# felixlutz/carla-social-force-model

Hardware: AMD Instinct MI355X
Metric: sfm_ticks_per_s (higher is better)
Workload: dtype f32

## Files before the change

### carla-social-force-model_amd/_lib.py

```python
from __future__ import annotations

import ctypes as C
import os

import numpy as np

PKG_DIR = os.path.dirname(os.path.abspath(__file__))
LIB_PATH = os.environ.get("SFM_LIB_PATH") or os.path.join(PKG_DIR, "libsfm_hip.so")
ABI_VERSION = 17
SINCE = {"sfm_step_packed": 4, "sfm_set_dynamic_obstacles_packed": 4, "sfm_step_records": 5,
         **{n: 6 for n in ("sfm_batch_create", "sfm_batch_destroy", "sfm_batch_set_stream", "sfm_batch_set_params",
                           "sfm_batch_upload_state", "sfm_batch_set_borders", "sfm_batch_set_static_obstacles",
                           "sfm_batch_set_dynamic_obstacles", "sfm_batch_tick", "sfm_batch_run", "sfm_batch_download_state",
                           "sfm_batch_last_error")},
         **{n: 7 for n in ("sfm_batch_set_waypoint_streams", "sfm_batch_download_waypoints", "sfm_batch_run_recorded")},
         **{n: 8 for n in ("sfm_batch_set_dynamic_boxes", "sfm_batch_download_dynamic_obstacles")},
         **{n: 9 for n in ("sfm_batch_set_mode_fsm", "sfm_batch_download_modes")},
         **{n: 10 for n in ("sfm_batch_tick_forces", "sfm_batch_run_recorded_forces")},
         **{n: 11 for n in ("sfm_batch_set_spawn_schedule", "sfm_batch_download_spawns")},
         **{n: 12 for n in ("sfm_batch_set_vehicle_tracks", "sfm_batch_download_vehicle_tracks")},
         **{n: 13 for n in ("sfm_batch_snapshot", "sfm_batch_restart")},
         **{n: 14 for n in ("sfm_batch_set_steering", "sfm_batch_set_commands", "sfm_batch_download_steering",
                            "sfm_batch_device_ptr")},
         **{n: 15 for n in ("sfm_batch_set_observation", "sfm_batch_observe", "sfm_batch_download_observations",
# ... 40 lines not shown
    "sfm_destroy": (C.c_int, [_H]),
    "sfm_set_params": (C.c_int, [_H, C.POINTER(SfmParamsC)]),
    "sfm_set_stream": (C.c_int, [_H, C.c_void_p]),
    "sfm_set_borders": (C.c_int, [_H, C.c_int, _I, _F, _F, _F, _F, _F]),
    "sfm_set_static_obstacles": (C.c_int, [_H, C.c_int, _I, _F, _F, _F, _F]),
    "sfm_set_dynamic_obstacles": (C.c_int, [_H, C.c_int, _I, _F, _F, _F, _F, _F, _F]),
    "sfm_set_dynamic_boxes": (C.c_int, [_H, C.c_int, _I, _F, _F, _F, _F, _F, _F, _F, _F]),
    "sfm_download_dynamic_obstacles": (C.c_int, [_H, _F, _F, _F, _F]),
    "sfm_upload_state": (C.c_int, [_H, C.c_int, _F, _F, _F, _F, _F, _F, _F, _F, _F, _F, _U8]),
    "sfm_set_shard": (C.c_int, [_H, C.c_int, C.c_int]),
    "sfm_set_waypoint_stream": (C.c_int, [_H, C.c_uint32, C.c_float, C.c_float]),
    "sfm_set_mode_fsm": (C.c_int, [_H, C.c_int, _U8, _F, _F, _F, _F, _F, _I, _F, _F, _U8, C.c_int, C.c_float, _F]),
    "sfm_download_modes": (C.c_int, [_H, _U8, _F, _I]),
    "sfm_tick": (C.c_int, [_H, C.c_uint32]),
    "sfm_run": (C.c_int, [_H, C.c_int, C.c_uint32]),
    "sfm_run_recorded": (C.c_int, [_H, C.c_int, C.c_uint32, C.c_int, _F, C.c_int, C.POINTER(C.c_int)]),
    "sfm_download_velocities": (C.c_int, [_H, _F, _F, _F]),
    "sfm_step_packed": (C.c_int, [_H, C.c_int, _F, _F, C.c_uint32, _F]),
    "sfm_step_records": (C.c_int, [_H, C.c_int, C.c_void_p, C.c_int64, _I, _U8, C.c_float, C.c_uint32, _F, C.POINTER(C.c_int32)]),
    "sfm_set_dynamic_obstacles_packed": (C.c_int, [_H, C.c_int, _I, _F, _F]),
    "sfm_download_state": (C.c_int, [_H, _F, _F, _F, _F, _F, _F, _F, _F]),
    "sfm_download_forces": (C.c_int, [_H, C.c_int, _F, _F, _F]),
    "sfm_get_arrived": (C.c_int, [_H, C.c_float, _U8]),
    "sfm_download_draw_counts": (C.c_int, [_H, _U32]),
    "sfm_packed_state_ptr": (C.c_void_p, [_H, C.POINTER(C.c_int)]),
    "sfm_packed_z_ptr": (C.c_void_p, [_H]),
    "sfm_row_data_ptr": (C.c_void_p, [_H, C.c_int, C.POINTER(C.c_int)]),
    "sfm_resort": (C.c_int, [_H]),
    "sfm_last_error": (C.c_char_p, [_H]),
    "sfm_get_timing": (C.c_int, [_H, C.POINTER(C.c_float), C.POINTER(C.c_int), C.POINTER(C.c_int)]),
    "sfm_set_timing": (C.c_int, [_H, C.c_int]),
    "sfm_profile_dominant_kernel": (C.c_int, [_H, C.c_int, C.POINTER(C.c_float)]),
    "sfm_kernel_variant": (C.c_char_p, [_H]),
    "sfm_get_pair_work": (C.c_int, [_H, C.POINTER(C.c_longlong), C.POINTER(C.c_longlong)]),
    "sfm_set_partition": (C.c_int, [_H, C.c_int, C.c_int, _I]),
    "sfm_tick_begin": (C.c_int, [_H, C.c_uint32]),
    "sfm_tick_end": (C.c_int, [_H, C.c_uint32]),
    "sfm_batch_create": (C.c_int, [C.c_int, C.POINTER(SfmParamsC), C.c_int, C.POINTER(_H)]),
    "sfm_batch_destroy": (C.c_int, [_H]),
    "sfm_batch_set_stream": (C.c_int, [_H, C.c_void_p]),
    "sfm_batch_set_params": (C.c_int, [_H, C.POINTER(SfmParamsC)]),
    "sfm_batch_upload_state": (C.c_int, [_H, _I, _F, _F, _F, _F, _F, _F, _F, _F, _F, _F, _U8]),
    "sfm_batch_set_borders": (C.c_int, [_H, _I, _I, _F, _F, _F, _F, _F]),
    "sfm_batch_set_static_obstacles": (C.c_int, [_H, _I, _I, _F, _F, _F, _F]),
    "sfm_batch_set_dynamic_obstacles": (C.c_int, [_H, _I, _I, _F, _F, _F, _F, _F, _F]),
    "sfm_batch_tick": (C.c_int, [_H, C.c_uint32]),
    "sfm_batch_run": (C.c_int, [_H, C.c_int, C.c_uint32]),
    "sfm_batch_download_state": (C.c_int, [_H, _F, _F, _F, _F, _F, _F]),
    "sfm_batch_last_error": (C.c_char_p, [_H]),
    "sfm_batch_set_waypoint_streams": (C.c_int, [_H, _U32, _F, _F]),
    "sfm_batch_download_waypoints": (C.c_int, [_H, _F, _F, _U32]),
    "sfm_batch_run_recorded": (C.c_int, [_H, C.c_int, C.c_uint32, C.c_int, _F, _F, C.c_int, C.POINTER(C.c_int)]),
    "sfm_batch_set_dynamic_boxes": (C.c_int, [_H, _I, _I, _F, _F, _F, _F, _F, _F, _F, _F]),
    "sfm_batch_download_dynamic_obstacles": (C.c_int, [_H, _F, _F, _F, _F]),
    "sfm_batch_set_mode_fsm": (C.c_int, [_H, _U8, _F, _F, _F, _F, _F, _I, _F, _F, _U8, _I, _F, _F, _F]),
    "sfm_batch_download_modes": (C.c_int, [_H, _U8, _F, _I, _F]),
    "sfm_batch_tick_forces": (C.c_int, [_H, C.c_uint32, C.c_uint32, _F]),
    "sfm_batch_run_recorded_forces": (C.c_int, [_H, C.c_int, C.c_uint32, C.c_int, C.c_uint32, _F, _F, _F, C.c_int,
                                                C.POINTER(C.c_int)]),
    "sfm_batch_set_spawn_schedule": (C.c_int, [_H, _F, _U8]),
    "sfm_batch_download_spawns": (C.c_int, [_H, _U8, _F]),
    "sfm_batch_set_vehicle_tracks": (C.c_int, [_H, _I, _I, _F, _F, _F, _F, _F, _F]),
    "sfm_batch_download_vehicle_tracks": (C.c_int, [_H, C.POINTER(C.c_int64), _U8]),
    "sfm_batch_snapshot": (C.c_int, [_H]),
    "sfm_batch_restart": (C.c_int, [_H, _U8]),
    "sfm_batch_set_steering": (C.c_int, [_H, _U8, _F, _F, _F]),
# ... 87 lines not shown
```

### carla-social-force-model_amd/csrc/sfm_capi.hip

```cpp
#include "sfm_capi_common.h"

using namespace sfm;

constexpr int GEO_SLICES_MAX = 16;


struct DevGeo {
    DevBuf<int> off;
    DevBuf<float2> pts;
    DevBuf<float4> ctr;
    DevBuf<float4> seg;
    int K = 0;
    int P = 0;
    PinnedBuf<char> stage;
    std::vector<int> off_host;
    bool lazy = false;
    bool lazy_off = false;
};

struct FsmDev {
    bool on = false;
    int n = 0;
    DevBuf<uint8_t> mode;
    DevBuf<float> target, initial, crossing, margin, next;
// ... 98 lines not shown
    FusedDev fused;
    int pair_geo_mode = -1;
    int fused_mode = -1;
    bool hosted = false;
    PinnedBuf<char> down_stage;
    std::vector<float> step_cols;
    std::vector<uint8_t> step_mask;
    bool used_fused = false;
    unsigned long long api_seq = 0, carry_seq = 0;
    bool carry_ok = false;
    int carry_sl = 0;
    bool last_list = false;

    uint32_t seed = 0;
    float world_side = 0.f, arrive_thr = 2.0f;

    FsmDev fsm;

    Event ev0, ev1;
    Stream aux;
    Event ev_fork, ev_join;
    bool overlap_geo = true;
    bool geo_ahead = false;
    DevBuf<uint32_t> work2;
    bool begin_done = false, begin_forked = false, last_split = false;
    int begin_geo_slices = 0;
    uint32_t begin_flags = 0;
    int timed_ticks = 0, timed_launches = 0;
    bool timing_valid = false;
    bool timing_on = true;
    int ipw_last = 0;
    int ipw_override = 0, team_override = 0;
    char variant[64] = "none";
};

static int fail(SfmHandle* h, int code, const char* msg) {
    if (h) h->err = msg; else g_create_error = msg;
    return code;
}

static int bind(SfmHandle* h) {
    if (!h) return SFM_ERR_INVALID;
    ++h->api_seq;
    hipError_t e = hipSetDevice(h->device);
    if (e != hipSuccess) { h->err = std::string("hipSetDevice: ") + hipGetErrorString(e); return SFM_ERR_HIP; }
    return SFM_OK;
}

static void drop_geo_ahead(SfmHandle* h) {
    if (h && h->geo_ahead) {
        hipStreamSynchronize(h->aux);
        h->geo_ahead = false;
    }
    if (h) h->begin_done = false;
}


extern "C" {

int sfm_abi_version(void) { return SFM_ABI_VERSION; }

int sfm_create(const SfmParams* params, int device_id, SfmHandle** out) {
    if (!out) return fail(nullptr, SFM_ERR_INVALID, "out is NULL");
    *out = nullptr;
    const char* why = nullptr;
    if (!check_params(params, &why)) return fail(nullptr, SFM_ERR_INVALID, why);
    int ndev = 0;
    hipError_t e = hipGetDeviceCount(&ndev);
    if (e != hipSuccess || ndev <= 0) return fail(nullptr, SFM_ERR_NO_DEVICE, "no HIP device visible (libsfm_hip needs an MI355X)");
    if (device_id < 0 || device_id >= ndev) return fail(nullptr, SFM_ERR_INVALID, "device_id out of range");
    e = hipSetDevice(device_id);
    if (e != hipSuccess) return fail(nullptr, SFM_ERR_HIP, hipGetErrorString(e));
    SfmHandle* h = new SfmHandle();
    h->device = device_id;
    h->prm = *params;
    if (h->ev0.create() != hipSuccess || h->ev1.create() != hipSuccess) {
        delete h;
        return fail(nullptr, SFM_ERR_HIP, "hipEventCreate failed");
    }
    if (h->aux.create(hipStreamNonBlocking) != hipSuccess || h->ev_fork.create(hipEventDisableTiming) != hipSuccess ||
        h->ev_join.create(hipEventDisableTiming) != hipSuccess) {
        h->aux.reset();
        h->overlap_geo = false;
    }
    const char* ov = getenv("SFM_IPW");
    if (ov) h->ipw_override = atoi(ov);
    ov = getenv("SFM_TEAM");
    if (ov) h->team_override = atoi(ov);
    ov = getenv("SFM_SYM");
    if (ov) h->sym_mode = atoi(ov);
    ov = getenv("SFM_CUTOFF");
    if (ov) h->cut_mode = atoi(ov);
    ov = getenv("SFM_PAIR_GEO");
    if (ov) h->pair_geo_mode = atoi(ov);
    ov = getenv("SFM_FUSED");
    if (ov) h->fused_mode = atoi(ov);
    ov = getenv("SFM_REORDER");
    if (ov) h->reorder_mode = atoi(ov);
    ov = getenv("SFM_GEO_SLICES");
    if (ov) h->geo_slices_override = std::min(GEO_SLICES_MAX, std::max(1, atoi(ov)));
    ov = getenv("SFM_STRIPS");
    if (ov) h->strips_override = atoi(ov) != 0 ? 1 : 0;
    ov = getenv("SFM_RESORT_EVERY");
    if (ov) { h->resort_every = atoi(ov); h->resort_every_set = true; }
    h->dpp_dir = probe_dpp_direction(nullptr);
    *out = h;
    return SFM_OK;
}

int sfm_destroy(SfmHandle* h) {
    if (!h) return SFM_OK;
    hipSetDevice(h->device);
    hipStreamSynchronize(h->stream);
    if (h->aux) hipStreamSynchronize(h->aux);
    delete h;
    return SFM_OK;
}

int sfm_set_params(SfmHandle* h, const SfmParams* params) {
    if (!h) return SFM_ERR_INVALID;
    const char* why = nullptr;
    if (!check_params(params, &why)) return fail(h, SFM_ERR_INVALID, why);
    drop_geo_ahead(h);
    h->carry_ok = false;
    h->prm = *params;
    return SFM_OK;
}

int sfm_set_stream(SfmHandle* h, void* hip_stream) {
// ... 603 lines not shown
    return sa;
}

constexpr int PHASE_FULL = 0, PHASE_BEGIN = 1, PHASE_END = 2;
constexpr int LIST_ALL = 0, LIST_OWN = 1, LIST_REMOTE = 2;

static int fused_launch(SfmHandle* h, uint32_t flags, int mode, int* sl) {
    const int n_g = (h->n_t + 1) / 2;
    const size_t rows = (size_t)n_g * (size_t)h->N_pad;
    TickArgs a;
    fill_args(h, a, flags);
    const bool geo = a.geo != nullptr;
    int slices = 0, nw = 16;
    const int n_pair = fused_pair_workgroups(n_g);
    if (geo) {
        slices = h->n_t <= 64 ? 4 : 2;
        if (h->n_t >= 6) slices = std::max(slices, std::min(FUSED_GEO_SLICES_MAX, (256 - n_pair) / h->n_t));
        if (n_pair + h->n_t * slices > 512) nw = 8;
    }
    const size_t grow = (size_t)FUSED_GEO_SLICES_MAX * (size_t)h->N_pad;
    if (geo && a.adv.M > 0) {
        float4* c_in = mode ? h->fused.dyn_ctr_alt : h->dynamics.ctr;
        float2* p_in = mode ? h->fused.dyn_pts_alt : h->dynamics.pts;
        a.dynamics.ctr = c_in; a.dynamics.pts = p_in;
        a.adv.ctr = c_in; a.adv.pts = p_in;
        a.adv.ctr_out = mode ? h->dynamics.ctr : h->fused.dyn_ctr_alt;
        a.adv.pts_out = mode ? h->dynamics.pts : h->fused.dyn_pts_alt;
    }
    const FusedArgs f{h->fused.fslab + (size_t)(*sl ^ 1) * rows, h->fused.fslab + (size_t)*sl * rows,
                      h->z3 ? h->fused.fslabz + (size_t)(*sl ^ 1) * rows : nullptr, h->z3 ? h->fused.fslabz + (size_t)*sl * rows : nullptr,
                      h->own, h->fused.own_alt, n_g, h->n_t, n_g % 8 == 0 ? 1 : 0,
                      geo ? h->fused.fgeo + (size_t)(*sl ^ 1) * grow : nullptr, geo ? h->fused.fgeo + (size_t)*sl * grow : nullptr, slices,
                      geo ? h->n_t * slices : 0, n_pair, mode};
    HIP_TRY(h, launch_fused_tick(h->rad, a, f, h->stream, nw));
    if (mode != 0) {
        h->cur ^= 1;
        swap(h->own, h->fused.own_alt);
        if (geo && a.adv.M > 0) {
            swap(h->dynamics.ctr, h->fused.dyn_ctr_alt);
            swap(h->dynamics.pts, h->fused.dyn_pts_alt);
        }
    }
    *sl ^= 1;
    return SFM_OK;
}

static int fused_reserve(SfmHandle* h) {
    const size_t need = (size_t)2 * (size_t)((h->n_t + 1) / 2) * (size_t)h->N_pad;
    FusedDev& f = h->fused;
    if (need > f.fslab.cap()) HIP_TRY(h, f.fslab.alloc(need));
    if (h->z3 && need > f.fslabz.cap()) HIP_TRY(h, f.fslabz.alloc(need));
    if (f.own_alt.cap() < (size_t)h->cap) HIP_TRY(h, f.own_alt.alloc((size_t)h->cap));
    const size_t gneed = (size_t)2 * FUSED_GEO_SLICES_MAX * (size_t)h->N_pad;
    if (gneed > f.fgeo.cap()) HIP_TRY(h, f.fgeo.alloc(gneed));
    if (h->dyn_boxes && h->dynamics.K > 0) {
        if (f.dyn_ctr_alt.cap() != h->dynamics.ctr.cap()) HIP_TRY(h, f.dyn_ctr_alt.alloc(h->dynamics.ctr.cap()));
        if (f.dyn_pts_alt.cap() != h->dynamics.pts.cap()) HIP_TRY(h, f.dyn_pts_alt.alloc(h->dynamics.pts.cap()));
    }
    return SFM_OK;
}

static int run_fused(SfmHandle* h, int ticks, uint32_t flags, bool carry, bool geo) {
    int rc = fused_reserve(h);
    if (rc) return rc;
    snprintf(h->variant, sizeof(h->variant), geo ? "sfm_fused_tick_kernel(geo)" : "sfm_fused_tick_kernel");
    if (h->timing_on) HIP_TRY(h, hipEventRecord(h->ev0, h->stream));
    int sl = carry ? h->carry_sl : 0;
// ... 655 lines not shown
    int rc = bind(h);
    if (rc) return rc;
    if (!h->pk[0]) return fail(h, SFM_ERR_STATE, "sfm_upload_state has not been called");
    if (!h->reordered || h->N == 0) return SFM_OK;
    if (h->fsm.on && !(h->i_begin == 0 && h->i_end == h->N))
        return fail(h, SFM_ERR_STATE, "sfm_resort on a shard with the device-side mode state machine");
    return resort_rows(h);
}

const char* sfm_last_error(const SfmHandle* h) { return h ? h->err.c_str() : g_create_error.c_str(); }

int sfm_set_timing(SfmHandle* h, int enable) {
    if (!h) return SFM_ERR_INVALID;
    h->carry_ok = false;
    h->timing_on = enable != 0;
    if (!h->timing_on) h->timing_valid = false;
    return SFM_OK;
}

int sfm_get_timing(SfmHandle* h, float* elapsed_ms, int* ticks, int* launches) {
    int rc = bind(h);
    if (rc) return rc;
    if (!h->timing_valid) return fail(h, SFM_ERR_STATE, h->timing_on ? "no timed run yet" : "timing is switched off (sfm_set_timing)");
    HIP_TRY(h, hipEventSynchronize(h->ev1));
    float ms = 0.f;
    HIP_TRY(h, hipEventElapsedTime(&ms, h->ev0, h->ev1));
    if (elapsed_ms) *elapsed_ms = ms;
    if (ticks) *ticks = h->timed_ticks;
    if (launches) *launches = h->timed_launches;
    return SFM_OK;
}

const char* sfm_kernel_variant(const SfmHandle* h) { return h ? h->variant : "none"; }

int sfm_get_pair_work(SfmHandle* h, long long* tile_pair_items, long long* pair_terms) {
    int rc = bind(h);
    if (rc) return rc;
    if (!h->pk[0]) return fail(h, SFM_ERR_STATE, "sfm_upload_state has not been called");
    if (!h->used_sym) return fail(h, SFM_ERR_STATE, "the last tick did not run the symmetric pair kernel");
    HIP_TRY(h, hipStreamSynchronize(h->stream));
    const long long t_own = (h->i_end + WAVE - 1) / WAVE - h->i_begin / WAVE;
    long long items, diag_items = (t_own + 1) / 2;
    if (h->last_list) {
        int cnt[4] = {0, 0, 0, 0};
        HIP_TRY(h, hipMemcpy(cnt, h->work_count, sizeof(int) * 4, hipMemcpyDeviceToHost));
        items = (h->count_zeroed ? cnt[2] : cnt[0]) + (h->last_split ? (h->count_zeroed ? cnt[3] : cnt[1]) : 0);
    } else {
        const long long n_t = h->n_t;
        items = n_t * (n_t - 1) / 2 + diag_items;
    }
    if (tile_pair_items) *tile_pair_items = items;
    if (pair_terms) *pair_terms = (items - diag_items) * (long long)(WAVE * WAVE) + t_own * (long long)(WAVE * WAVE / 2);
    return SFM_OK;
}

}
```

### carla-social-force-model_amd/csrc/sfm_capi_common.h

```cpp
#pragma once
#include "sfm_devbuf.h"
#include "sfm_device.h"
#include "sfm_hip.h"

#include <algorithm>
#include <cmath>
#include <numeric>
#include <cstdio>
#include <cstdlib>
#include <cstring>
#include <limits>
#include <string>
#include <vector>

namespace sfm {
hipError_t launch_tick(int ipw, int team, bool z3, bool rad, const TickArgs& a, hipStream_t st);
hipError_t launch_arrived(const float4* pk, const float4* own, int N, float thr2, uint8_t* mask, hipStream_t st);
hipError_t launch_sym_list(const TickArgs& a, const SymArgs& sa, hipStream_t st, int partners = 0, bool count_is_zero = false);
hipError_t launch_sym_pair(bool rad, const TickArgs& a, const SymArgs& sa, hipStream_t st);
hipError_t launch_sym_epilogue(bool rad, const TickArgs& a, const SymArgs& sa, hipStream_t st);
hipError_t launch_fused_tick(bool rad, const TickArgs& a, const FusedArgs& f, hipStream_t st, int waves);
int fused_pair_workgroups(int n_g);
hipError_t launch_sym_pair_geo(bool rad, const TickArgs& a, const SymArgs& sa, hipStream_t st);
int sym_item_count(int n_t);
hipError_t launch_strip_bounds(const float4* box, const float* vmax, int n_t, int tps, int n_strips, float4* sbox, float* svmax,
                               hipStream_t st);
hipError_t launch_tile_strip_bounds(const float4* pk, int N, int n_t, int tps, int n_strips, float4* box, float* vmax, float4* sbox,
                                    float* svmax, hipStream_t st);
hipError_t launch_geometry(bool rad, const TickArgs& a, hipStream_t st);
hipError_t launch_modes(const TickArgs& a, hipStream_t st);
struct ReorderBufs { unsigned long long *key64_in, *key64_out; uint32_t *row_a, *row_b, *key32_in, *key32_out; void* temp; size_t temp_bytes; };
size_t reorder_temp_bytes(int N);
hipError_t launch_resort(const float4* pk, int N, int strip_rows, const ReorderBufs& b, hipStream_t st);
hipError_t launch_resort_blocks(const float4* pk, int N, const BlockPlan& pl, const ReorderBufs& b, hipStream_t st);
hipError_t launch_unpack_geo(const char* block, float4* ctr, int K, float2* pts, int P, int* off, bool with_off, hipStream_t st);
hipError_t launch_unpack_rows(const char* block, size_t b_own, size_t b_zv, size_t b_rr, size_t b_cm, int n_pad, float4* pk0,
                              float4* pk1, float4* own, float2* zv0, float2* zv1, float* radius, uint8_t* crossing, uint32_t* draws,
                              const char* geo_block, float4* ctr, int K, float2* pts, int P, int* off, bool with_off, hipStream_t st);
hipError_t launch_gather(const uint32_t* src, int N, const float4* pk_in, float4* pk_out, const float2* zv_in, float2* zv_out,
                         const float4* own_in, float4* own_out, const float* rad_in, float* rad_out, const uint8_t* cr_in,
                         uint8_t* cr_out, const uint32_t* dr_in, uint32_t* dr_out, const uint32_t* id_in, uint32_t* id_out,
                         hipStream_t st);
hipError_t launch_tile_bounds(const float4* pk, const float2* zv, int N, float4* box, float* vmax, hipStream_t st, int t_lo = 0,
                              int t_hi = -1);
int probe_dpp_direction(hipStream_t st);
hipError_t launch_batch_tick(bool z3, bool ext, bool modes, bool spawn, bool steer, const BatchArgs& a, int B, hipStream_t st);
hipError_t launch_batch_park_unborn(const int* scene_off, const uint8_t* born, float4* pk, float2* zv, int B, hipStream_t st);
hipError_t launch_batch_place_tracks(const BatchTracks& t, const int* off, const float2* local, float4* ctr, float2* pts, int M,
                                     hipStream_t st);
hipError_t launch_batch_restart(const BatchRestart& r, int scenes, hipStream_t st);
hipError_t launch_batch_restart_noise(const RestartNoiseArgs& a, int scenes, hipStream_t st);
hipError_t launch_batch_observe(const ObserveArgs& a, int B, hipStream_t st);
hipError_t launch_batch_episode(const EpisodeArgs& a, int B, hipStream_t st);
hipError_t launch_batch_scan(const ScanArgs& a, int B, hipStream_t st);
// ... 42 lines not shown
```

### carla-social-force-model_amd/csrc/sfm_device.h

```cpp
#pragma once
#include <hip/hip_runtime.h>
#include <stdint.h>

namespace sfm {

constexpr int WAVE = 64;
constexpr int BLOCK = 256;
constexpr int WAVES_PER_BLOCK = BLOCK / WAVE;
constexpr int TILE_J = BLOCK;
constexpr float TINY = 1e-30f;
constexpr float COINCIDENT_RINV = 1e14f;

constexpr float FAR_AWAY = 3.0e15f;
constexpr float FAR_STEP = 1.0e12f;
constexpr float BOX_LIMIT = 1.0e14f;
constexpr float NEAR_LIMIT = 1.0e12f;

struct IxConst {
    float lam;
    float eg;
    float c1;
    float k1;
    float k2;
    float negA;
// ... 115 lines not shown
    int zero_count;
    uint32_t* idx;
    uint32_t row_base;
    uint32_t cap_pairs;
    struct SpillArgs* spill;
    int tick_serial;
};

struct SpillArgs {
    long long* ovf;
    int n_pad;
    int tick;
};

constexpr int FUSED_GEO_SLICES_MAX = 8;
struct alignas(16) FusedArgs {
    const float2* slab_prev;
    float2* slab_next;
    const float* slabz_prev;
    float* slabz_next;
    const float4* own_cur;
    float4* own_next;
    int n_g;
    int n_t;
    int blocked;
    const float2* geo_prev;
    float2* geo_next;
    int geo_slices;
    int n_geo_wg;
    int n_pair_wg;
    int mode;
};

constexpr int BATCH_MAX_N = 1024;
struct BatchParams {
    IxConst ped, stat, dyn;
    float border_a, border_nlb;
    float inv_tau, dt, max_speed_factor;
    int en_acc, en_ped, en_border, en_static, en_dynamic;
    int rad;
    int pad;
};
struct BatchGeo {
    const int* item_off;
    const int* off;
    const float2* pts;
    const float4* ctr;
};
struct BatchStream {
    uint32_t seed;
    float world_side;
    float arrive_thr2;
    float pad;
};
struct BatchModeScene {
    float arrive_thr2;
    float veh_ext_x, veh_ext_y;
    int despawn_on_arrival;
};
struct BatchModes {
    uint8_t* mode;
    float* target;
    const float4* speeds;
    const int* wp_off;
    const float2* wp_xy;
    const uint8_t* wp_cross;
// ... 163 lines not shown
```

### carla-social-force-model_amd/csrc/sfm_kernels.hip

```cpp
#include "sfm_device.h"
#include "sfm_interaction.h"

#include <algorithm>
#include <type_traits>

namespace sfm {

typedef float v2f __attribute__((ext_vector_type(2)));
__device__ __forceinline__ v2f bcast(float v) { v2f r; r.x = v; r.y = v; return r; }
template <bool RAD, bool CUT>
__device__ __forceinline__ bool moussaid_planar_pk(const IxConst& c, v2f pj, v2f uj, v2f Ti, v2f Ui, float rsum, float reach2, v2f& term) {
    const v2f dd = pj - Ti;
    const float d2 = fmaf(dd.x, dd.x, dd.y * dd.y);
    if (CUT && !__any(!(d2 > reach2))) return false;
    v2f sq, rr;
    sq.x = d2;
    rr.x = rsq(d2);
    const v2f Dv = __builtin_elementwise_fma(dd, __builtin_shufflevector(rr, rr, 0, 0), Ui - uj);
    const float D2 = fmaf(Dv.x, Dv.x, fmaf(Dv.y, Dv.y, TINY));
    sq.y = D2;
    rr.y = rsq(D2);
    const float rD = rr.y;
    float aL = 0.f;
    if (CUT) {
// ... 1939 lines not shown
    } else if (p < GROUP) {
#pragma unroll
        for (int k = 0; k < NW / 2; ++k) { const float3 u = fi(tl * (NW / 2) + k); r.x += u.x; r.y += u.y; r.z += u.z; }
        row = GY;
    } else {
#pragma unroll
        for (int h = 0; h < 2; ++h)
#pragma unroll
            for (int k = 0; k < NW / 4; ++k) { const float3 u = fj((2 * h + tl) * (NW / 4) + k); r.x += u.x; r.y += u.y; r.z += u.z; }
        row = GX;
    }
    f.slab_next[(size_t)row * a.N_pad + i] = make_float2(r.x, r.y);
    if (Z3) f.slabz_next[(size_t)row * a.N_pad + i] = r.z;
}

__global__ __launch_bounds__(BLOCK) void sfm_dynamic_boxes_kernel(float4* __restrict__ ctr, const int* __restrict__ off,
                                                                  const float2* __restrict__ local, const float2* __restrict__ rot,
                                                                  float2* __restrict__ pts, int M, float dt, int advance) {
    const int k = blockIdx.x * WAVES_PER_BLOCK + (int)(threadIdx.x >> 6);
    if (k >= M) return;
    advance_vehicle(DynAdvance{ctr, off, local, rot, pts, M, dt, 0, nullptr, nullptr}, k, threadIdx.x & (WAVE - 1), advance != 0);
}

__global__ void sfm_arrived_kernel(const float4* __restrict__ pk, const float4* __restrict__ own, int N, float thr2,
                                   uint8_t* __restrict__ mask) {
    const int i = blockIdx.x * blockDim.x + threadIdx.x;
    if (i >= N) return;
    const float4 s = pk[i];
    const float4 o = own[i];
    const float ddx = o.x - s.x, ddy = o.y - s.y;
    mask[i] = fmaf(ddx, ddx, ddy * ddy) < thr2 ? 1 : 0;
}

template <int IPW, bool Z3, bool RAD, int TEAM>
static hipError_t launch_one(const TickArgs& a, hipStream_t st) {
    const int n_local = a.i_end - a.i_begin;
    if (n_local <= 0) return hipSuccess;
    const int per_block = IPW * (WAVES_PER_BLOCK / TEAM);
    const int grid = (n_local + per_block - 1) / per_block;
    TickArgs b = a;
    b.adv.block0 = grid;
    const int extra = a.adv.M > 0 ? (a.adv.M + WAVES_PER_BLOCK - 1) / WAVES_PER_BLOCK : 0;
    hipLaunchKernelGGL((sfm_tick_kernel<IPW, Z3, RAD, TEAM>), dim3(grid + extra), dim3(BLOCK), 0, st, b);
    return hipGetLastError();
}

template <bool Z3, bool RAD, int TEAM>
static hipError_t launch_ipw(int ipw, const TickArgs& a, hipStream_t st) {
    switch (ipw) {
        case 1: return launch_one<1, Z3, RAD, TEAM>(a, st);
        case 2: return launch_one<2, Z3, RAD, TEAM>(a, st);
        case 4: return launch_one<4, Z3, RAD, TEAM>(a, st);
        default: return launch_one<8, Z3, RAD, TEAM>(a, st);
    }
}

template <int TEAM>
static hipError_t launch_team(int ipw, bool z3, bool rad, const TickArgs& a, hipStream_t st) {
    if (z3) return rad ? launch_ipw<true, true, TEAM>(ipw, a, st) : launch_ipw<true, false, TEAM>(ipw, a, st);
    return rad ? launch_ipw<false, true, TEAM>(ipw, a, st) : launch_ipw<false, false, TEAM>(ipw, a, st);
}

hipError_t launch_tick(int ipw, int team, bool z3, bool rad, const TickArgs& a, hipStream_t st) {
    return team == 4 ? launch_team<4>(ipw, z3, rad, a, st) : launch_team<1>(ipw, z3, rad, a, st);
}

// ... 115 lines not shown
}

hipError_t launch_sym_epilogue(bool rad, const TickArgs& a, const SymArgs& sa, hipStream_t st) {
    if (a.N <= 0) return hipSuccess;
    const bool thin = sa.n_t >= 1024;
    if (rad) { if (thin) launch_sym_epilogue_t<true, 4>(a, sa, st); else launch_sym_epilogue_t<true, EPI_WAVES>(a, sa, st); }
    else { if (thin) launch_sym_epilogue_t<false, 4>(a, sa, st); else launch_sym_epilogue_t<false, EPI_WAVES>(a, sa, st); }
    return hipGetLastError();
}

int fused_pair_workgroups(int n_g) { return (n_g + 1) / 2 + n_g * ((n_g - 1) / 2) + ((n_g & 1) ? 0 : n_g / 2); }

template <bool RAD, int NW>
static void launch_fused_t(dim3 grid, bool geo, bool z3, const TickArgs& a, const FusedArgs& f, hipStream_t st) {
    if (z3) {
        if (geo) hipLaunchKernelGGL((sfm_fused_tick_kernel<RAD, NW, true, true>), grid, dim3(NW * WAVE), 0, st, a, f);
        else hipLaunchKernelGGL((sfm_fused_tick_kernel<RAD, NW, true, false>), grid, dim3(NW * WAVE), 0, st, a, f);
    } else {
        if (geo) hipLaunchKernelGGL((sfm_fused_tick_kernel<RAD, NW, false, true>), grid, dim3(NW * WAVE), 0, st, a, f);
        else hipLaunchKernelGGL((sfm_fused_tick_kernel<RAD, NW, false, false>), grid, dim3(NW * WAVE), 0, st, a, f);
    }
}

hipError_t launch_fused_tick(bool rad, const TickArgs& a, const FusedArgs& f, hipStream_t st, int nw) {
    if (a.N <= 1 || f.n_g < 1) return hipErrorInvalidValue;
    const bool geo = f.n_geo_wg > 0, z3 = f.slabz_next != nullptr;
    const int n_adv = (geo && a.adv.M > 0) ? (a.adv.M + nw - 1) / nw : 0;
    const dim3 grid(f.n_geo_wg + f.n_pair_wg + n_adv);
    if (nw == 8) { if (rad) launch_fused_t<true, 8>(grid, geo, z3, a, f, st); else launch_fused_t<false, 8>(grid, geo, z3, a, f, st); }
    else { if (rad) launch_fused_t<true, 16>(grid, geo, z3, a, f, st); else launch_fused_t<false, 16>(grid, geo, z3, a, f, st); }
    return hipGetLastError();
}

int probe_dpp_direction(hipStream_t st) {
    int* d = nullptr;
    if (hipMalloc(reinterpret_cast<void**>(&d), 64 * sizeof(int)) != hipSuccess) return 0;
    hipLaunchKernelGGL(sfm_dpp_probe_kernel, dim3(1), dim3(64), 0, st, d);
    int h[64];
    hipError_t e = hipMemcpy(h, d, sizeof(h), hipMemcpyDeviceToHost);
    hipFree(d);
    if (e != hipSuccess) return 0;
    bool up = true, down = true;
    for (int l = 0; l < 64; ++l) { up &= (h[l] == ((l + 1) & 63)); down &= (h[l] == ((l + 63) & 63)); }
    return up ? 1 : (down ? -1 : 0);
}

hipError_t launch_dynamic_boxes(float4* ctr, const int* off, const float2* local, const float2* rot, float2* pts, int M,
                                float dt, int advance, hipStream_t st) {
    if (M <= 0) return hipSuccess;
    hipLaunchKernelGGL(sfm_dynamic_boxes_kernel, dim3((M + WAVES_PER_BLOCK - 1) / WAVES_PER_BLOCK), dim3(BLOCK), 0, st, ctr, off, local,
                       rot, pts, M, dt, advance);
    return hipGetLastError();
}

hipError_t launch_arrived(const float4* pk, const float4* own, int N, float thr2, uint8_t* mask, hipStream_t st) {
    if (N <= 0) return hipSuccess;
    hipLaunchKernelGGL(sfm_arrived_kernel, dim3((N + 255) / 256), dim3(256), 0, st, pk, own, N, thr2, mask);
    return hipGetLastError();
}

}
```

### carla-social-force-model_amd/engine.py

```python
from __future__ import annotations

import ctypes as C

import numpy as np

from . import _lib
from ._lib import FORCE_NAMES, FORCE_TOTAL, SfmLibraryError, f32, fptr, iptr, u8ptr


def interaction_from_table(tbl):
    return _lib.SfmInteraction(tbl.get("lambda", 2.0), tbl.get("A", 4.5), tbl.get("gamma", 0.35),
                               tbl.get("n", 2.0), tbl.get("n_prime", 3.0), tbl.get("epsilon", 0.005),
                               tbl.get("perception_threshold", 20))


def params_from_config(sfm_config, step_length, honour_file_keys=False):
    act = sfm_config["forces"]
    p = _lib.SfmParamsC()
    p.use_ped_radius = int(bool(sfm_config.get("use_ped_radius", False)))
    p.max_speed_factor = sfm_config.get("max_speed_factor", 1.3)
    p.tau = sfm_config.get("goal_force", {}).get("tau", 0.5)
    if honour_file_keys:
        p.max_speed_factor = sfm_config.get("max_speed_multiplier", p.max_speed_factor)
        p.tau = sfm_config.get("acceleration_force", {}).get("tau", p.tau)
# ... 326 lines not shown

    def packed_state_ptr(self):
        npad = C.c_int(0)
        p = self._lib.sfm_packed_state_ptr(self._h, C.byref(npad))
        return p, npad.value

    def packed_z_ptr(self):
        return self._lib.sfm_packed_z_ptr(self._h)

    def row_data_ptr(self, which):
        b = C.c_int(0)
        p = self._lib.sfm_row_data_ptr(self._h, int(which), C.byref(b))
        return p, b.value

    def resort(self):
        self._check(self._lib.sfm_resort(self._h), "sfm_resort")

    def set_timing(self, enable):
        self._check(self._lib.sfm_set_timing(self._h, 1 if enable else 0), "sfm_set_timing")

    def timing(self):
        ms, t, l = C.c_float(0), C.c_int(0), C.c_int(0)
        self._check(self._lib.sfm_get_timing(self._h, C.byref(ms), C.byref(t), C.byref(l)), "sfm_get_timing")
        return ms.value, t.value, l.value

    def profile_dominant_kernel(self, reps=100):
        us = C.c_float(0)
        self._check(self._lib.sfm_profile_dominant_kernel(self._h, int(reps), C.byref(us)), "sfm_profile_dominant_kernel")
        return us.value

    def kernel_variant(self):
        return self._lib.sfm_kernel_variant(self._h).decode()

    def pair_work(self):
        items, terms = C.c_longlong(0), C.c_longlong(0)
        self._check(self._lib.sfm_get_pair_work(self._h, C.byref(items), C.byref(terms)), "sfm_get_pair_work")
        return items.value, terms.value
```

### include/sfm_hip.h

```cpp
#ifndef SFM_HIP_H
#define SFM_HIP_H

#include <stdint.h>

#ifdef __cplusplus
extern "C" {
#endif

#define SFM_ABI_VERSION 17

typedef struct SfmHandle SfmHandle;

typedef enum SfmStatus {
    SFM_OK = 0,
    SFM_ERR_INVALID = -1,
    SFM_ERR_HIP = -2,
    SFM_ERR_STATE = -3,
    SFM_ERR_NO_DEVICE = -4
} SfmStatus;

enum { SFM_FORCE_ACCELERATION = 0, SFM_FORCE_PEDESTRIAN = 1, SFM_FORCE_BORDER = 2,
       SFM_FORCE_STATIC_OBSTACLE = 3, SFM_FORCE_DYNAMIC_OBSTACLE = 4, SFM_NUM_FORCES = 5,
       SFM_FORCE_TOTAL = 5 };

// ... 59 lines not shown


int sfm_tick(SfmHandle* h, uint32_t flags);
int sfm_run(SfmHandle* h, int ticks, uint32_t flags);
int sfm_tick_begin(SfmHandle* h, uint32_t flags);
int sfm_tick_end(SfmHandle* h, uint32_t flags);

int sfm_run_recorded(SfmHandle* h, int ticks, uint32_t flags, int stride, float* frames, int max_frames, int* n_frames);


int sfm_download_velocities(SfmHandle* h, float* vx, float* vy, float* vz);
int sfm_step_packed(SfmHandle* h, int N, const float* rows, const float* zvz, uint32_t flags, float* v_out);
int sfm_step_records(SfmHandle* h, int N, const void* records, int64_t stride, const int32_t* field_offsets, const uint8_t* border_off,
                     float planar_tolerance, uint32_t flags, float* v_out, int32_t* was_planar);

int sfm_download_state(SfmHandle* h, float* x, float* y, float* z, float* vx, float* vy, float* vz,
                       float* wx, float* wy);
int sfm_download_forces(SfmHandle* h, int which, float* fx, float* fy, float* fz);
int sfm_get_arrived(SfmHandle* h, float threshold, uint8_t* mask);
int sfm_download_draw_counts(SfmHandle* h, uint32_t* counts);


void* sfm_packed_state_ptr(SfmHandle* h, int* n_pad);
void* sfm_packed_z_ptr(SfmHandle* h);
void* sfm_row_data_ptr(SfmHandle* h, int which, int* bytes_per_row);
int sfm_resort(SfmHandle* h);


const char* sfm_last_error(const SfmHandle* h);
int sfm_get_timing(SfmHandle* h, float* elapsed_ms, int* ticks, int* launches);
int sfm_set_timing(SfmHandle* h, int enable);
int sfm_profile_dominant_kernel(SfmHandle* h, int reps, float* avg_us);
const char* sfm_kernel_variant(const SfmHandle* h);
int sfm_get_pair_work(SfmHandle* h, long long* tile_pair_items, long long* pair_terms);
int sfm_abi_version(void);


#define SFM_BATCH_MAX_N 1024
typedef struct SfmBatch SfmBatch;

int sfm_batch_create(int B, const SfmParams* params, int device_id, SfmBatch** out);
int sfm_batch_destroy(SfmBatch* b);
int sfm_batch_set_stream(SfmBatch* b, void* hip_stream);
int sfm_batch_set_params(SfmBatch* b, const SfmParams* params);
int sfm_batch_upload_state(SfmBatch* b, const int32_t* scene_off, const float* x, const float* y, const float* z,
                           const float* vx, const float* vy, const float* vz, const float* wx, const float* wy,
                           const float* target_speed, const float* radius, const uint8_t* crossing_mask);
int sfm_batch_set_borders(SfmBatch* b, const int32_t* scene_item_off, const int32_t* offsets, const float* px, const float* py,
                          const float* cx, const float* cy, const float* cull_len);
int sfm_batch_set_static_obstacles(SfmBatch* b, const int32_t* scene_item_off, const int32_t* offsets, const float* px,
                                   const float* py, const float* cx, const float* cy);
int sfm_batch_set_dynamic_obstacles(SfmBatch* b, const int32_t* scene_item_off, const int32_t* offsets, const float* px,
                                    const float* py, const float* cx, const float* cy, const float* vx, const float* vy);
int sfm_batch_set_dynamic_boxes(SfmBatch* b, const int32_t* scene_item_off, const int32_t* offsets, const float* ux,
                                const float* uy, const float* cx, const float* cy, const float* yaw_cos, const float* yaw_sin,
                                const float* vx, const float* vy);
int sfm_batch_download_dynamic_obstacles(SfmBatch* b, float* cx, float* cy, float* px, float* py);
#define SFM_BATCH_MAX_TRACK_KEYS (1 << 22)
int sfm_batch_set_vehicle_tracks(SfmBatch* b, const int32_t* trk_off, const int32_t* first_tick, const float* kx, const float* ky,
                                 const float* kvx, const float* kvy, const float* kcos, const float* ksin);
int sfm_batch_download_vehicle_tracks(SfmBatch* b, int64_t* tick, uint8_t* present);
int sfm_batch_tick(SfmBatch* b, uint32_t flags);
int sfm_batch_run(SfmBatch* b, int ticks, uint32_t flags);
int sfm_batch_set_waypoint_streams(SfmBatch* b, const uint32_t* seed, const float* world_side, const float* arrive_threshold);
int sfm_batch_download_waypoints(SfmBatch* b, float* wx, float* wy, uint32_t* draws);
#define SFM_BATCH_MAX_RECORD_BYTES (1ull << 30)
// ... 77 lines not shown
```

Baseline: 64070.

## Add lean specialized fused tick kernel for pedestrian-only blocked layouts

Adds a compile-time specialized fused tick kernel for the common case with no radius, no geometry slices, and group counts that are multiples of 8 up to 32. It uses a compact 128-byte argument struct, a fixed 16-wave schedule, and templated sizes so loops and slab reductions unroll. Pair forces are computed from a shared-memory transposed layout, and a fallback recomputes rows whose forces are non-finite. The aim is to cut argument loading, register pressure and general-path branching in the dominant per-tick kernel. The trade-off is a second code path that must match the general kernel's results.

```diff
diff --git a/carla-social-force-model_amd/_lib.py b/carla-social-force-model_amd/_lib.py
--- a/carla-social-force-model_amd/_lib.py
+++ b/carla-social-force-model_amd/_lib.py
@@ -96,6 +96,7 @@
     "sfm_set_timing": (C.c_int, [_H, C.c_int]),
     "sfm_profile_dominant_kernel": (C.c_int, [_H, C.c_int, C.POINTER(C.c_float)]),
     "sfm_kernel_variant": (C.c_char_p, [_H]),
+    "sfm_fused_form": (C.c_char_p, [_H]),
     "sfm_get_pair_work": (C.c_int, [_H, C.POINTER(C.c_longlong), C.POINTER(C.c_longlong)]),
     "sfm_set_partition": (C.c_int, [_H, C.c_int, C.c_int, _I]),
     "sfm_tick_begin": (C.c_int, [_H, C.c_uint32]),
diff --git a/carla-social-force-model_amd/csrc/sfm_capi.hip b/carla-social-force-model_amd/csrc/sfm_capi.hip
--- a/carla-social-force-model_amd/csrc/sfm_capi.hip
+++ b/carla-social-force-model_amd/csrc/sfm_capi.hip
@@ -154,6 +154,8 @@
     int ipw_last = 0;
     int ipw_override = 0, team_override = 0;
     char variant[64] = "none";
+    bool fused_lean = true;
+    bool fused_lean_ran = false;
 };
 
 static int fail(SfmHandle* h, int code, const char* msg) {
@@ -217,6 +219,8 @@
     if (ov) h->pair_geo_mode = atoi(ov);
     ov = getenv("SFM_FUSED");
     if (ov) h->fused_mode = atoi(ov);
+    ov = getenv("SFM_FUSED_LEAN");
+    if (ov) h->fused_lean = atoi(ov) != 0;
     ov = getenv("SFM_REORDER");
     if (ov) h->reorder_mode = atoi(ov);
     ov = getenv("SFM_GEO_SLICES");
@@ -886,7 +890,9 @@
                       h->own, h->fused.own_alt, n_g, h->n_t, n_g % 8 == 0 ? 1 : 0,
                       geo ? h->fused.fgeo + (size_t)(*sl ^ 1) * grow : nullptr, geo ? h->fused.fgeo + (size_t)*sl * grow : nullptr, slices,
                       geo ? h->n_t * slices : 0, n_pair, mode};
-    HIP_TRY(h, launch_fused_tick(h->rad, a, f, h->stream, nw));
+    h->fused_lean_ran = h->fused_lean && fused_lean_takes(h->rad, a, f);
+    if (h->fused_lean_ran) HIP_TRY(h, launch_fused_tick_lean(a, f, h->stream));
+    else HIP_TRY(h, launch_fused_tick(h->rad, a, f, h->stream, nw));
     if (mode != 0) {
         h->cur ^= 1;
         swap(h->own, h->fused.own_alt);
@@ -1608,6 +1614,10 @@
 }
 
 const char* sfm_kernel_variant(const SfmHandle* h) { return h ? h->variant : "none"; }
+const char* sfm_fused_form(const SfmHandle* h) {
+    if (!h || !h->used_fused) return "none";
+    return h->fused_lean_ran ? "sfm_fused_tick_kernel<lean>" : "sfm_fused_tick_kernel<general>";
+}
 
 int sfm_get_pair_work(SfmHandle* h, long long* tile_pair_items, long long* pair_terms) {
     int rc = bind(h);
diff --git a/carla-social-force-model_amd/csrc/sfm_capi_common.h b/carla-social-force-model_amd/csrc/sfm_capi_common.h
--- a/carla-social-force-model_amd/csrc/sfm_capi_common.h
+++ b/carla-social-force-model_amd/csrc/sfm_capi_common.h
@@ -20,6 +20,8 @@
 hipError_t launch_sym_pair(bool rad, const TickArgs& a, const SymArgs& sa, hipStream_t st);
 hipError_t launch_sym_epilogue(bool rad, const TickArgs& a, const SymArgs& sa, hipStream_t st);
 hipError_t launch_fused_tick(bool rad, const TickArgs& a, const FusedArgs& f, hipStream_t st, int waves);
+bool fused_lean_takes(bool rad, const TickArgs& a, const FusedArgs& f);
+hipError_t launch_fused_tick_lean(const TickArgs& a, const FusedArgs& f, hipStream_t st);
 int fused_pair_workgroups(int n_g);
 hipError_t launch_sym_pair_geo(bool rad, const TickArgs& a, const SymArgs& sa, hipStream_t st);
 int sym_item_count(int n_t);
diff --git a/carla-social-force-model_amd/csrc/sfm_device.h b/carla-social-force-model_amd/csrc/sfm_device.h
--- a/carla-social-force-model_amd/csrc/sfm_device.h
+++ b/carla-social-force-model_amd/csrc/sfm_device.h
@@ -171,6 +171,25 @@
     int mode;
 };
 
+constexpr uint32_t LEAN_EN_ACC = 0x100u, LEAN_EN_PED = 0x200u, LEAN_INTEGRATE = 0x400u;
+struct alignas(16) LeanTickArgs {
+    const float4* pk_cur;
+    float4* pk_next;
+    const float4* own_cur;
+    float4* own_next;
+    const float2* slab_prev;
+    float2* slab_next;
+    uint32_t* draws;
+    const uint32_t* ids;
+    IxConst ped;
+    float inv_tau, dt, max_speed_factor, arrive_thr2;
+    uint32_t seed;
+    float world_side;
+    uint32_t bits;
+    uint32_t pad;
+};
+static_assert(sizeof(LeanTickArgs) == 128, "the lean fused tick's arguments: two 64-byte scalar loads");
+
 constexpr int BATCH_MAX_N = 1024;
 struct BatchParams {
     IxConst ped, stat, dyn;
diff --git a/carla-social-force-model_amd/csrc/sfm_kernels.hip b/carla-social-force-model_amd/csrc/sfm_kernels.hip
--- a/carla-social-force-model_amd/csrc/sfm_kernels.hip
+++ b/carla-social-force-model_amd/csrc/sfm_kernels.hip
@@ -1995,6 +1995,276 @@
     mask[i] = fmaf(ddx, ddx, ddy * ddy) < thr2 ? 1 : 0;
 }
 
+struct LeanShared {
+    float4 st[2 * GROUP];
+    float2 q[8][2 * GROUP];
+    float2 part[2 * GROUP];
+    int badrow[2 * GROUP];
+    int any;
+    float2 fi[16][WAVE];
+    float2 fj[16][WAVE];
+    float4 trav[4][2 * WAVE];
+};
+
+namespace lean {
+
+template <int N_G>
+__global__ __launch_bounds__(16 * WAVE, 8) void sfm_fused_tick_kernel(const LeanTickArgs a) {
+    constexpr int NW = 16, PARTS = 8, SPW = 4 * WAVE / NW, D = NW / 8, HALF = SPW / 2;
+    constexpr int N = N_G * GROUP;
+    constexpr int PER = N_G / PARTS;
+    static_assert(N_G % 8 == 0 && N_G >= 8 && N_G <= 32, "the lean form takes 8, 16, 24 or 32 groups");
+    __shared__ __attribute__((aligned(16))) char smem[sizeof(LeanShared)];
+    LeanShared& sh = *reinterpret_cast<LeanShared*>(smem);
+    const int tid = threadIdx.x;
+    const int lane = tid & (WAVE - 1);
+    const int wave = uniform(tid >> 6);
+    const bool en_acc = (a.bits & LEAN_EN_ACC) != 0, en_ped = (a.bits & LEAN_EN_PED) != 0, integrate = (a.bits & LEAN_INTEGRATE) != 0;
+    int GX, GY;
+    bool diag_item;
+    {
+        constexpr int s = N_G >> 2;
+        const int bid = (int)blockIdx.x;
+        const int x = bid & 7;
+        int k = bid >> 3;
+        if (x < 6) {
+            const int I = x < 3 ? 0 : (x < 5 ? 1 : 2), J = x < 3 ? x + 1 : (x < 5 ? x - 1 : 3);
+            GX = I * s + k / s;
+            GY = J * s + k % s;
+            diag_item = false;
+        } else {
+            constexpr int per_band = (s * s) >> 1;
+            const int I = 2 * (x - 6) + (k >= per_band ? 1 : 0);
+            if (k >= per_band) k -= per_band;
+            if (k < (s >> 1)) {
+                GX = I * s + 2 * k; GY = GX + 1;
+                diag_item = true;
+            } else {
+                int t = k - (s >> 1), u = 0;
+                while (t >= s - 1 - u) { t -= s - 1 - u; ++u; }
+                GX = I * s + u; GY = I * s + u + 1 + t;
+                diag_item = false;
+            }
+        }
+    }
+
+    const int quarter = wave & 3;
+    const int p = quarter * WAVE + lane;
+    const bool lower = wave < 4;
+    const int G = (quarter < 2) ? GX : GY;
+    const int i = G * GROUP + (quarter & 1) * WAVE + lane;
+    float4 st = make_float4(0.f, 0.f, 0.f, 0.f), o = st;
+    uint32_t nd0 = 0, pid = 0;
+    if (lower) {
+        st = a.pk_cur[i];
+        if (integrate) {
+            o = a.own_cur[i];
+            if ((a.bits & 2u) && diag_item) { nd0 = a.draws[i]; pid = a.ids ? a.ids[i] : (uint32_t)i; }
+        }
+    }
+    if (tid == 0) sh.any = 0;
+    {
+        const int pp = (wave & 1) * WAVE + lane;
+        const int part = wave >> 1;
+        const int Gq = (wave & 1) ? GY : GX;
+        float4 acc4 = make_float4(0.f, 0.f, 0.f, 0.f);
+        if (integrate && en_ped) {
+            constexpr uint32_t ROW = N * sizeof(float2);
+            const char* rows = reinterpret_cast<const char*>(a.slab_prev) + (uint32_t)(part * PER) * ROW;
+            const uint32_t at = (uint32_t)(Gq * (GROUP / 2) + lane) * (uint32_t)sizeof(float4);
+            auto col = [&](int k) {
+                uint32_t ro = (uint32_t)k * ROW;
+                asm("" : "+s"(ro));
+                return *reinterpret_cast<const float4*>(rows + ro + at);
+            };
+            if (PER == 4) {
+                const float4 v0 = col(0), v1 = col(1), v2 = col(2), v3 = col(3);
+                __builtin_amdgcn_sched_barrier(0);
+                acc4 = make_float4((v0.x + v1.x) + (v2.x + v3.x), (v0.y + v1.y) + (v2.y + v3.y),
+                                   (v0.z + v1.z) + (v2.z + v3.z), (v0.w + v1.w) + (v2.w + v3.w));
+            } else {
+                float4 v[8];
+#pragma unroll
+                for (int k = 0; k < 8; ++k) v[k] = (k < PER) ? col(k < PER ? k : 0) : make_float4(0.f, 0.f, 0.f, 0.f);
+                __builtin_amdgcn_sched_barrier(0);
+                acc4.x += ((v[0].x + v[1].x) + (v[2].x + v[3].x)) + ((v[4].x + v[5].x) + (v[6].x + v[7].x));
+                acc4.y += ((v[0].y + v[1].y) + (v[2].y + v[3].y)) + ((v[4].y + v[5].y) + (v[6].y + v[7].y));
+                acc4.z += ((v[0].z + v[1].z) + (v[2].z + v[3].z)) + ((v[4].z + v[5].z) + (v[6].z + v[7].z));
+                acc4.w += ((v[0].w + v[1].w) + (v[2].w + v[3].w)) + ((v[4].w + v[5].w) + (v[6].w + v[7].w));
+            }
+        }
+        sh.q[part][2 * pp] = make_float2(acc4.x, acc4.y);
+        sh.q[part][2 * pp + 1] = make_float2(acc4.z, acc4.w);
+    }
+    __syncthreads();
+    auto put_state = [&](const float4 ns) {
+        sh.st[p] = ns;
+        const float4 t = make_float4(ns.x, ns.y, a.ped.lam * ns.z, a.ped.lam * ns.w);
+        float* pl = reinterpret_cast<float*>(sh.trav) + (p >> 6) * 2 * WAVE + (p & (WAVE - 1));
+        pl[0] = t.x; pl[WAVE] = t.x;
+        pl[8 * WAVE] = t.y; pl[9 * WAVE] = t.y;
+        pl[16 * WAVE] = t.z; pl[17 * WAVE] = t.z;
+        pl[24 * WAVE] = t.w; pl[25 * WAVE] = t.w;
+    };
+    auto finish = [&](const float2 g) {
+        const float fpx = en_ped ? a.ped.negA * g.x : 0.f, fpy = en_ped ? a.ped.negA * g.y : 0.f;
+        const float x = st.x, y = st.y, vx = st.z, vy = st.w, ts = o.z;
+        float wx = o.x, wy = o.y;
+        float fax = 0.f, fay = 0.f, faz = 0.f;
+        if (en_acc) acceleration_force<false, true>(a, wx, wy, x, y, vx, vy, 0.f, ts, fax, fay, faz);
+        const float Fx = (fax + fpx) + 0.f, Fy = (fay + fpy) + 0.f;
+        float nvx, nvy, nvz;
+        capped_velocity<false, true>(a, vx, vy, 0.f, Fx, Fy, 0.f, ts, nvx, nvy, nvz);
+        float nx = x, ny = y;
+        if (a.bits & 1u) { nx = fmaf(a.dt, nvx, x); ny = fmaf(a.dt, nvy, y); }
+        const float4 ns = make_float4(nx, ny, nvx, nvy);
+        if (diag_item) {
+            if (a.bits & 2u) {
+                const float ax_ = wx - x, ay_ = wy - y;
+                if (fmaf(ax_, ax_, ay_ * ay_) < a.arrive_thr2) {
+                    const uint32_t nd = nd0 + 1u;
+                    const float2 w = next_waypoint(a.seed, pid, nd, a.world_side);
+                    wx = w.x; wy = w.y;
+                    a.draws[i] = nd;
+                }
+            }
+            a.own_next[i] = make_float4(wx, wy, o.z, o.w);
+            a.pk_next[i] = ns;
+        }
+        put_state(ns);
+    };
+    bool bad = false;
+    if (lower) {
+        if (integrate) {
+            float2 g = sh.q[0][p];
+#pragma unroll
+            for (int k = 1; k < PARTS; ++k) { const float2 q = sh.q[k][p]; g.x += q.x; g.y += q.y; }
+            bad = en_ped && (!(fabsf(g.x) < __builtin_inff()) || !(fabsf(g.y) < __builtin_inff()));
+            if (bad) sh.any = 1; else finish(g);
+        } else {
+            put_state(st);
+        }
+        sh.badrow[p] = bad ? 1 : 0;
+    }
+    __syncthreads();
+    if (sh.any) {
+        for (int q = wave; q < 2 * GROUP; q += NW) {
+            if (!sh.badrow[q]) continue;
+            const int Gq = (q < GROUP) ? GX : GY;
+            const int ip = Gq * GROUP + (q & (GROUP - 1));
+            const float4 si = a.pk_cur[ip];
+            const float xi = uniform(si.x), yi = uniform(si.y), vxi = uniform(si.z), vyi = uniform(si.w);
+            float gx = 0.f, gy = 0.f;
+            for (int j0 = 0; j0 < N; j0 += WAVE) {
+                const int j = j0 + lane;
+                const float4 pj = a.pk_cur[j];
+                float cx = 0.f, cy = 0.f, cz = 0.f, rinv;
+                moussaid<false, false, true>(a.ped, pj.x - xi, pj.y - yi, 0.f, vxi - pj.z, vyi - pj.w, 0.f, 0.f, cx, cy, cz, rinv);
+                const bool valid = j != ip;
+                gx += valid ? cx : 0.f;
+                gy += valid ? cy : 0.f;
+            }
+            gx = wave_sum(gx);
+            gy = wave_sum(gy);
+            if (lane == 0) sh.part[q] = make_float2(gx, gy);
+        }
+        __syncthreads();
+        if (bad) finish(sh.part[p]);
+        __syncthreads();
+    }
+
+    int ia, ib, sig0;
+    bool diag = false;
+    if (diag_item) {
+        const int sel = wave / (NW / 2);
+        const int lw = wave % (NW / 2);
+        const int base = sel * GROUP;
+        if (lw < 2 * D) {
+            ia = ib = base + (lw / D) * WAVE;
+            sig0 = 1 + (lw % D) * SPW;
+            diag = true;
+        } else {
+            ia = base; ib = base + WAVE;
+            sig0 = (lw - 2 * D) * SPW;
+        }
+    } else {
+        const int q = wave / (NW / 4);
+        ia = (q >> 1) * WAVE;
+        ib = GROUP + (q & 1) * WAVE;
+        sig0 = (wave % (NW / 4)) * SPW;
+    }
+    float fxi = 0.f, fyi = 0.f, fxb = 0.f, fyb = 0.f;
+    const IxConst& c = a.ped;
+    const float4 pj = sh.st[ib + lane];
+    const float ujx = c.lam * pj.z, ujy = c.lam * pj.w;
+    const int s0 = diag ? 1 + ((sig0 - 1) >> 1) : sig0 >> 1;
+    const float* pl = reinterpret_cast<const float*>(sh.trav) + (ia >> 6) * 2 * WAVE + lane + s0;
+    v2f fjx = bcast(0.f), fjy = bcast(0.f);
+    auto chain = [&](auto xb_tag) __attribute__((always_inline)) {
+        constexpr int XB = decltype(xb_tag)::value;
+        const bool tail_one_sided = diag && (s0 + XB + HALF - 1 == 32);
+        v2f X, Y, U, V;
+        X.x = pl[0]; X.y = pl[XB]; Y.x = pl[8 * WAVE]; Y.y = pl[8 * WAVE + XB];
+        U.x = pl[16 * WAVE]; U.y = pl[16 * WAVE + XB]; V.x = pl[24 * WAVE]; V.y = pl[24 * WAVE + XB];
+#pragma unroll
+        for (int s_ = 0; s_ < HALF; ++s_) {
+            v2f Xn = X, Yn = Y, Un = U, Vn = V;
+            if (s_ + 1 < HALF) {
+                Xn.x = pl[s_ + 1]; Xn.y = pl[s_ + 1 + XB]; Yn.x = pl[8 * WAVE + s_ + 1]; Yn.y = pl[8 * WAVE + s_ + 1 + XB];
+                Un.x = pl[16 * WAVE + s_ + 1]; Un.y = pl[16 * WAVE + s_ + 1 + XB]; Vn.x = pl[24 * WAVE + s_ + 1]; Vn.y = pl[24 * WAVE + s_ + 1 + XB];
+            }
+            __builtin_amdgcn_sched_barrier(0);
+            v2f cx, cy;
+            moussaid_planar_x2<false>(c, pj.x, pj.y, ujx, ujy, X, Y, U, V, cx, cy, bcast(0.f));
+            fxi = rot_in(fxi) + cx.x; fyi = rot_in(fyi) + cy.x;
+            fxb = rot_in(fxb) + cx.y; fyb = rot_in(fyb) + cy.y;
+            if (s_ + 1 == HALF && tail_one_sided) { fjx.x -= cx.x; fjy.x -= cy.x; }
+            else { fjx -= cx; fjy -= cy; }
+            X = Xn; Y = Yn; U = Un; V = Vn;
+            __builtin_amdgcn_sched_barrier(0);
+        }
+        const int from = ((lane - XB) & (WAVE - 1)) << 2;
+        fxi += __int_as_float(__builtin_amdgcn_ds_bpermute(from, __float_as_int(fxb)));
+        fyi += __int_as_float(__builtin_amdgcn_ds_bpermute(from, __float_as_int(fyb)));
+    };
+    if (diag) chain(std::integral_constant<int, 16>{});
+    else chain(std::integral_constant<int, 32>{});
+    sh.fi[wave][(lane + s0 + HALF - 1) & (WAVE - 1)] = make_float2(fxi, fyi);
+    sh.fj[wave][lane] = make_float2(fjx.x + fjx.y, fjy.x + fjy.y);
+    __syncthreads();
+    if (!lower) return;
+    const int tl = (p >> 6) & 1, l = lane;
+    float2 r = make_float2(0.f, 0.f);
+    int row;
+    if (diag_item) {
+        const int w0 = (p < GROUP) ? 0 : NW / 2;
+#pragma unroll
+        for (int k = 0; k < D; ++k) {
+            const float2 u = sh.fi[w0 + tl * D + k][l], v = sh.fj[w0 + tl * D + k][l];
+            r.x += u.x + v.x; r.y += u.y + v.y;
+        }
+#pragma unroll
+        for (int k = 0; k < 2 * D; ++k) {
+            const float2 u = tl ? sh.fj[w0 + 2 * D + k][l] : sh.fi[w0 + 2 * D + k][l];
+            r.x += u.x; r.y += u.y;
+        }
+        row = G;
+    } else if (p < GROUP) {
+#pragma unroll
+        for (int k = 0; k < NW / 2; ++k) { const float2 u = sh.fi[tl * (NW / 2) + k][l]; r.x += u.x; r.y += u.y; }
+        row = GY;
+    } else {
+#pragma unroll
+        for (int h = 0; h < 2; ++h)
+#pragma unroll
+            for (int k = 0; k < NW / 4; ++k) { const float2 u = sh.fj[(2 * h + tl) * (NW / 4) + k][l]; r.x += u.x; r.y += u.y; }
+        row = GX;
+    }
+    a.slab_next[(uint32_t)row * (uint32_t)N + (uint32_t)i] = r;
+}
+
+}
+
 template <int IPW, bool Z3, bool RAD, int TEAM>
 static hipError_t launch_one(const TickArgs& a, hipStream_t st) {
     const int n_local = a.i_end - a.i_begin;
@@ -2176,6 +2446,26 @@
     return hipGetLastError();
 }
 
+bool fused_lean_takes(bool rad, const TickArgs& a, const FusedArgs& f) {
+    return !rad && !f.slabz_next && f.n_geo_wg == 0 && f.blocked && f.n_g <= 32 && f.n_g % 8 == 0 && a.N == f.n_g * GROUP && a.N_pad == a.N &&
+           f.n_t == 2 * f.n_g;
+}
+
+hipError_t launch_fused_tick_lean(const TickArgs& a, const FusedArgs& f, hipStream_t st) {
+    if (!fused_lean_takes(false, a, f)) return hipErrorInvalidValue;
+    LeanTickArgs l{a.pk_cur, a.pk_next, f.own_cur, f.own_next, f.slab_prev, f.slab_next, a.draws, a.ids, a.ped,
+                   a.inv_tau, a.dt, a.max_speed_factor, a.arrive_thr2, a.seed, a.world_side,
+                   (a.flags & 3u) | (a.en_acc ? LEAN_EN_ACC : 0u) | (a.en_ped ? LEAN_EN_PED : 0u) | (f.mode != 0 ? LEAN_INTEGRATE : 0u), 0u};
+    const dim3 grid(f.n_pair_wg), block(16 * WAVE);
+    switch (f.n_g) {
+        case 8: hipLaunchKernelGGL((lean::sfm_fused_tick_kernel<8>), grid, block, 0, st, l); break;
+        case 16: hipLaunchKernelGGL((lean::sfm_fused_tick_kernel<16>), grid, block, 0, st, l); break;
+        case 24: hipLaunchKernelGGL((lean::sfm_fused_tick_kernel<24>), grid, block, 0, st, l); break;
+        default: hipLaunchKernelGGL((lean::sfm_fused_tick_kernel<32>), grid, block, 0, st, l); break;
+    }
+    return hipGetLastError();
+}
+
 int probe_dpp_direction(hipStream_t st) {
     int* d = nullptr;
     if (hipMalloc(reinterpret_cast<void**>(&d), 64 * sizeof(int)) != hipSuccess) return 0;
diff --git a/carla-social-force-model_amd/engine.py b/carla-social-force-model_amd/engine.py
--- a/carla-social-force-model_amd/engine.py
+++ b/carla-social-force-model_amd/engine.py
@@ -382,6 +382,9 @@
     def kernel_variant(self):
         return self._lib.sfm_kernel_variant(self._h).decode()
 
+    def fused_form(self):
+        return self._lib.sfm_fused_form(self._h).decode()
+
     def pair_work(self):
         items, terms = C.c_longlong(0), C.c_longlong(0)
         self._check(self._lib.sfm_get_pair_work(self._h, C.byref(items), C.byref(terms)), "sfm_get_pair_work")
diff --git a/include/sfm_hip.h b/include/sfm_hip.h
--- a/include/sfm_hip.h
+++ b/include/sfm_hip.h
@@ -115,6 +115,7 @@
 int sfm_set_timing(SfmHandle* h, int enable);
 int sfm_profile_dominant_kernel(SfmHandle* h, int reps, float* avg_us);
 const char* sfm_kernel_variant(const SfmHandle* h);
+const char* sfm_fused_form(const SfmHandle* h);
 int sfm_get_pair_work(SfmHandle* h, long long* tile_pair_items, long long* pair_terms);
 int sfm_abi_version(void);
 
```

Result: faster. 66180, median of 6 (+3.3%).
